# Sohojoe/ppo-dash

Measured on AMD Instinct MI355X. Metric: env-steps/sec (rollout+GAE+PPO update) at 4096 envs×128 steps, 1/2/4/8 MI355X, higher is better.
Workload: dtype f32

## Files before the change

### ppo-dash_amd/csrc/gemm.hip

```cpp
#include "igemm.h"
#include "igemm_x9.h"
#include "small.h"

namespace {
constexpr int IMG = 84, IMG2 = 84 * 84;
constexpr int C1S = 7104;
static_assert(C1S >= IMG2 && (C1S / 2) % 64 == 32, "conv1 stage channel stride");

template <typename InT, class C_>
struct Conv1Fwd : C_ {
  using BCtx = typename C_::BCtx;
  const InT* obs; const int64_t* idx; long long row0; int C, M;
  const float* w; const float* bias; float* out;
  struct ACtx { const InT* base; bool ok; };
  __device__ ACtx a_ctx(int m, int) const {
    if (m >= M) return {obs, false};
    const int b = m / 400, pp = m - b * 400, oy = pp / 20, ox = pp - oy * 20;
    return {obs + obs_row(idx, row0, b) * (long long)(C * IMG2) + (oy * 4) * IMG + ox * 4, true};
  }
  using Raw = std::conditional_t<sizeof(InT) == 1, uint32_t, f32x4>;
  __device__ Raw a_load(const ACtx& c, int k) const {
    if (!c.ok) return Raw{};
    const int ch = k >> 6, ky = (k >> 3) & 7, kx = k & 7;
    return *reinterpret_cast<const Raw*>(c.base + ch * IMG2 + ky * IMG + kx);
// ... 401 lines not shown
__device__ __forceinline__ void conv2_fwd_x9c_body(const float* __restrict__ a1, int B,
                                                   const uint16_t* __restrict__ wpl, const float* __restrict__ bias,
                                                   float* __restrict__ out, uint16_t* __restrict__ mbits,
                                                   uint8_t* __restrict__ lds) {
  constexpr int U = 400, PLN = 4 * U, STG = 3 * PLN, KS = 8, WN = 64 * 512;
  static_assert(MT == 5 || MT == 6, "row tiles: 6, or 5 with the lone pixel elsewhere");
  constexpr int UNITS = 4 * U, UPER = (UNITS + 511) / 512;
  static_assert(STG == C2F_STG, "stage size");
  bf16x8* const S = reinterpret_cast<bf16x8*>(lds);
  int (*const vtab)[16] = reinterpret_cast<int (*)[16]>(lds + 2 * STG * 16);
  int (*const otab)[16] = reinterpret_cast<int (*)[16]>(lds + 2 * STG * 16 + MT * 16 * 4);
  const int tid = threadIdx.x, lane = tid & 63, wave = tid >> 6, i16 = lane & 15, g = lane >> 4;
  const int nt = wave & 3, kh = wave >> 2, co = 16 * nt + i16;
  if (tid < 16) {
    int t = 0;
    for (int v = tid; v <= 88; v += 16)
      if (v % 10 != 9 && t < MT) {
        vtab[t][tid] = v;
        otab[t][tid] = 9 * (v / 10) + v % 10;
        ++t;
      }
    if (MT == 5 && t == 4) {
      const int v = 82 + (tid - 9);
      vtab[4][tid] = v;
      otab[4][tid] = 9 * (v / 10) + v % 10;
      t = 5;
    }
    for (; t < MT; ++t) {
      vtab[t][tid] = tid;
      otab[t][tid] = -1;
    }
  }
  bf16x8 bw[KS][3];
#pragma unroll
  for (int s = 0; s < KS; ++s)
#pragma unroll
    for (int p = 0; p < 3; ++p)
      bw[s][p] = *reinterpret_cast<const bf16x8*>(wpl + (size_t)p * WN + co * 512 + (8 * kh + s) * 32 + 8 * g);
  const f32x4 bv4 = *reinterpret_cast<const f32x4*>(bias + 16 * nt + 4 * g);
  wait_vm0();
  int usrc[UPER], udst[UPER];
#pragma unroll
  for (int j = 0; j < UPER; ++j) {
    const int u = min(tid + 512 * j, UNITS - 1), rho = 8 * (u >> 5) + (u & 7), c = (u >> 3) & 3;
    const int par = rho / 100, rem = rho - 100 * par, yh = rem / 10, xh = rem - 10 * yh;
    const int y = 2 * yh + (par >> 1), x = 2 * xh + (par & 1);
    usrc[j] = (y * 20 + x) * 8 + 2 * c;
    udst[j] = c * U + rho;
  }
  const bool has_last = tid + 512 * (UPER - 1) < UNITS;
  f32x4 stg[UPER][2];
  bf16x8 lo[UPER];
  auto fetch_unit = [&](int b, int j) {
    if constexpr ((DBG & 4) != 0) {
      asm volatile("" : "+v"(stg[j][0]), "+v"(stg[j][1]));
      return;
    }
    const f32x4* src = reinterpret_cast<const f32x4*>(a1 + (size_t)b * 12800);
    stg[j][0] = src[usrc[j]];
    stg[j][1] = src[usrc[j] + 1];
  };
  auto fetch = [&](int b) {
#pragma unroll
    for (int j = 0; j < UPER; ++j) fetch_unit(b, j);
  };
  auto put_hm = [&](int j, int st) {
    if constexpr ((DBG & 2) != 0) {
      asm volatile("" ::"v"(stg[j][0]), "v"(stg[j][1]));
      return;
    }
    Frag3 f;
    split8(stg[j][0], stg[j][1], f, NP == 1);
    lo[j] = f.l;
    if (j < UPER - 1 || has_last) {
      bf16x8* d = S + st * STG + udst[j];
      d[0] = f.h;
      if constexpr (NP > 1) d[PLN] = f.m;
    }
  };
  auto put_l = [&](int j, int st) {
    if constexpr ((DBG & 2) != 0) return;
    if constexpr (NP > 1)
      if (j < UPER - 1 || has_last) S[st * STG + 2 * PLN + udst[j]] = lo[j];
  };
  auto lds_barrier = []() { asm volatile("s_waitcnt lgkmcnt(0)\n\ts_barrier" ::: "memory"); };
  __syncthreads();
  int vrow[MT];
#pragma unroll
  for (int t = 0; t < MT; ++t) vrow[t] = vtab[t][i16] + g * U;
  const int G = gridDim.x;
  int b = blockIdx.x, cur = 0;
  if (b < B) {
    fetch(b);
#pragma unroll
    for (int j = 0; j < UPER; ++j) {
      put_hm(j, 0);
      put_l(j, 0);
    }
    fetch(b + G < B ? b + G : b);
  }
  __syncthreads();
  for (; b < B; b += G) {
    const int bnn = b + 2 * G < B ? b + 2 * G : b;
    const bf16x8* Sc = S + cur * STG;
    f32x4 acc[MT];
#pragma unroll
    for (int t = 0; t < MT; ++t) acc[t] = zero4();
#pragma unroll
    for (int s = 0; s < KS; ++s) {
      const int tap = 8 * kh + s, ky = tap >> 2, kx = tap & 3;
      const int toff = 100 * (2 * (ky & 1) + (kx & 1)) + 10 * (ky >> 1) + (kx >> 1);
      const Frag3 w = {bw[s][0], bw[s][1], bw[s][2]};
#pragma unroll
      for (int t0 = 0; t0 < MT; t0 += 3) {
        Frag3 a[3];
#pragma unroll
        for (int u = 0; u < 3; ++u) {
          if (t0 + u >= MT) continue;
          const bf16x8* q = Sc + vrow[t0 + u] + toff;
          a[u].h = q[0];
          if constexpr (NP > 1) {
            a[u].m = q[PLN];
            a[u].l = q[2 * PLN];
          }
        }
#define PPO_PART(X, Y) \
  _Pragma("unroll") for (int u = 0; u < 3; ++u) if (t0 + u < MT) acc[t0 + u] = mma(w.Y, a[u].X, acc[t0 + u]);
        if constexpr ((DBG & 1) == 0) {
          PPO_PRODUCTS(NP, PPO_PART)
        } else {
#pragma unroll
          for (int u = 0; u < 3; ++u)
            if (t0 + u < MT) asm volatile("" ::"v"(a[u].h), "v"(a[u].m), "v"(a[u].l));
        }
#undef PPO_PART
      }
      if (s < UPER) put_hm(s, cur ^ 1);
      if (s >= 1 && s <= UPER) fetch_unit(bnn, s - 1);
      if (s == 5) lds_barrier();
      if (s >= 6) {
#pragma unroll
        for (int j = 0; j < UPER; ++j)
          if ((j & 1) == s - 6) put_l(j, cur ^ 1);
      }
    }
    lds_barrier();
    f32x4* R = reinterpret_cast<f32x4*>(S + cur * STG + 2 * PLN);
    if (kh == 1) {
#pragma unroll
      for (int t = 0; t < MT; ++t) R[(nt * MT + t) * 64 + lane] = acc[t];
    }
    lds_barrier();
    if (kh == 0) {
      const auto rs = make_rsrc(out + (size_t)b * (81 * 64), 81 * 64 * 4);
#pragma unroll
      for (int t = 0; t < MT; ++t) {
        const f32x4 v = acc[t] + R[(nt * MT + t) * 64 + lane];
        const int m = otab[t][i16];
        f32x4 y;
#pragma unroll
        for (int r = 0; r < 4; ++r) y[r] = fmaxf(v[r] + bv4[r], 0.f);
        if constexpr ((DBG & 8) == 0) bstore_f32x4(y, rs, m >= 0 ? 4 * (m * 64 + 16 * nt + 4 * g) : -1);
        if constexpr (MASK && (DBG & 8) == 0) {
          int nib = 0;
#pragma unroll
          for (int r = 0; r < 4; ++r) nib |= (y[r] > 0.f ? 1 : 0) << r;
          const int w16 = nib | (__shfl_down(nib, 16, 64) << 4) | (__shfl_down(nib, 32, 64) << 8) |
                          (__shfl_down(nib, 48, 64) << 12);
          if (g == 0 && m >= 0) mbits[((size_t)b * 81 + m) * 4 + nt] = (uint16_t)w16;
        }
      }
    }
    cur ^= 1;
  }
  if constexpr (MT == 5 && LONE) {
    __syncthreads();
    const int blk = blockIdx.x;
    const int nimg = blk < B ? (B - 1 - blk) / G + 1 : 0;
    conv2_lone_tiles<NP, MASK>(a1, bw, bias, out, mbits, lds, blk, G, nimg, 0, 1);
  }
}

#ifndef C2F_LONE
#define C2F_LONE 1
#endif
template <int NP, bool MASK = false, int DBG = 0>
__global__ __launch_bounds__(512) void conv2_fwd_x9c_kernel(const float* __restrict__ a1, int B,
                                                           const uint16_t* __restrict__ wpl,
                                                           const float* __restrict__ bias,
                                                           float* __restrict__ out,
                                                           uint16_t* __restrict__ mbits) {
  __shared__ __attribute__((aligned(16))) uint8_t lds[C2F_LDS];
  conv2_fwd_x9c_body<NP, MASK, DBG, C2F_LONE ? 5 : 6, C2F_LONE == 2>(a1, B, wpl, bias, out, mbits, lds);
}

constexpr int C2L_IR = 65;
constexpr int C2L_PL = 16 * C2L_IR;
constexpr int C2L_LDS = 2 * 3 * C2L_PL * 16 + 4 * 64 * 16;
static_assert(C2L_LDS <= C2F_LDS, "the lone tiles reuse the image loop's LDS");
template <int NP, bool MASK>
__device__ __forceinline__ void conv2_lone_tiles(const float* __restrict__ a1, const bf16x8 (&bw)[8][3],
                                                 const float* __restrict__ bias, float* __restrict__ out,
                                                 uint16_t* __restrict__ mbits, uint8_t* __restrict__ lds,
                                                 long long base, long long stride, int nimg, int t0, int tstep) {
  constexpr int KS = 8, M = 72, IR = C2L_IR, PL = C2L_PL;
  uint4 (*const P)[3 * PL] = reinterpret_cast<uint4 (*)[3 * PL]>(lds);
  f32x4* const R = reinterpret_cast<f32x4*>(lds + 2 * 3 * PL * 16);
  const int tid = threadIdx.x, lane = tid & 63, i16 = lane & 15, g = lane >> 4;
  const int wave = __builtin_amdgcn_readfirstlane(tid >> 6);
  const int nt = wave & 3, kh = wave >> 2;
  const int ntile = (nimg + 15) / 16;
  f32x4 pc[2][2];
  auto fetch = [&](int T) {
#pragma unroll
    for (int j = 0; j < 2; ++j) {
      const int c = tid + 512 * j, im = c >> 6, u = c & 63, i = 16 * T + im;
      const bool live = T < ntile && i < nimg;
      const float* src = a1 + (size_t)(base + stride * (live ? i : 0)) * 12800 + (16 + (u >> 4)) * 640 + (u & 15) * 8;
      pc[j][0] = live ? *reinterpret_cast<const f32x4*>(src) : zero4();
      pc[j][1] = live ? *reinterpret_cast<const f32x4*>(src + 4) : zero4();
    }
  };
  auto put = [&](int st) {
#pragma unroll
    for (int j = 0; j < 2; ++j) {
      const int c = tid + 512 * j, o = (c >> 6) * IR + (c & 63);
      Frag3 f;
      split8(pc[j][0], pc[j][1], f, NP == 1);
      P[st][o] = __builtin_bit_cast(uint4, f.h);
      if constexpr (NP != 1) {
        P[st][PL + o] = __builtin_bit_cast(uint4, f.m);
        P[st][2 * PL + o] = __builtin_bit_cast(uint4, f.l);
      }
    }
  };
  fetch(t0);
  put(0);
  __syncthreads();
  int cur = 0;
  for (int T = t0; T < ntile; T += tstep) {
    fetch(T + tstep);
    const int i = 16 * T + i16;
    const bool live = i < nimg;
    const long long b = base + stride * (long long)i;
    f32x4 acc = zero4();
#pragma unroll
    for (int s = 0; s < KS; ++s) {
      const int o = i16 * IR + (8 * kh + s) * 4 + g;
      Frag3 a;
      a.h = __builtin_bit_cast(bf16x8, P[cur][o]);
      if constexpr (NP != 1) {
        a.m = __builtin_bit_cast(bf16x8, P[cur][PL + o]);
        a.l = __builtin_bit_cast(bf16x8, P[cur][2 * PL + o]);
      }
      const Frag3 w = {bw[s][0], bw[s][1], bw[s][2]};
#define PPO_PART(X, Y) acc = mma(w.Y, a.X, acc);
      PPO_PRODUCTS(NP, PPO_PART)
#undef PPO_PART
    }
    if (kh == 1) R[nt * 64 + lane] = acc;
    put(cur ^ 1);
    __syncthreads();
    if (kh == 0) {
      const f32x4 bv4 = *reinterpret_cast<const f32x4*>(bias + 16 * nt + 4 * g);
      const f32x4 v = acc + R[nt * 64 + lane];
      f32x4 y;
#pragma unroll
      for (int r = 0; r < 4; ++r) y[r] = fmaxf(v[r] + bv4[r], 0.f);
      if (live) *reinterpret_cast<f32x4*>(out + (size_t)b * (81 * 64) + M * 64 + 16 * nt + 4 * g) = y;
      if constexpr (MASK) {
        int nib = 0;
#pragma unroll
        for (int r = 0; r < 4; ++r) nib |= (y[r] > 0.f ? 1 : 0) << r;
        const int w16 = nib | (__shfl_down(nib, 16, 64) << 4) | (__shfl_down(nib, 32, 64) << 8) |
                        (__shfl_down(nib, 48, 64) << 12);
        if (g == 0 && live) mbits[((size_t)b * 81 + M) * 4 + nt] = (uint16_t)w16;
      }
    }
    __syncthreads();
    cur ^= 1;
  }
}

template <int NP, bool MASK>
__global__ __launch_bounds__(512) void conv2_fwd_lone_kernel(const float* __restrict__ a1, int B,
                                                             const uint16_t* __restrict__ wpl,
                                                             const float* __restrict__ bias,
                                                             float* __restrict__ out,
                                                             uint16_t* __restrict__ mbits) {
  constexpr int KS = 8, WN = 64 * 512;
  __shared__ __attribute__((aligned(16))) uint8_t lds[C2L_LDS];
  const int tid = threadIdx.x, i16 = tid & 15, g = (tid & 63) >> 4, wave = tid >> 6;
  const int co = 16 * (wave & 3) + i16, kh = wave >> 2;
  bf16x8 bw[KS][3];
#pragma unroll
  for (int s = 0; s < KS; ++s)
#pragma unroll
    for (int p = 0; p < 3; ++p)
      bw[s][p] = *reinterpret_cast<const bf16x8*>(wpl + (size_t)p * WN + co * 512 + (8 * kh + s) * 32 + 8 * g);
  conv2_lone_tiles<NP, MASK>(a1, bw, bias, out, mbits, lds, 0, 1, B, blockIdx.x, gridDim.x);
}

__device__ __forceinline__ int c2w_pix(int r) {
  r = r < 80 ? r : 80;
  return r < 72 ? (r >> 3) * 9 + (r & 7) : (r - 72) * 9 + 8;
}

template <int NP, int DBG = 0>
__global__ __launch_bounds__(512) void conv2_wgrad_x9_kernel(const float* __restrict__ dz2,
                                                            const float* __restrict__ a1, int B,
                                                            float* __restrict__ slab,
                                                            float* __restrict__ slab_bias) {
  constexpr int XPL = 400 * 32, DR = 112, DPL = 64 * DR;
  constexpr int XU = 1600, XPER = (XU + 511) / 512, DU = 64 * 12, DPER = (DU + 511) / 512;
  __shared__ __attribute__((aligned(16))) uint16_t X[3 * XPL];
  __shared__ __attribute__((aligned(16))) uint16_t D[3 * DPL];
  __shared__ float bred[512];
  const int tid = threadIdx.x, lane = tid & 63, wave = tid >> 6, i16 = lane & 15, g = lane >> 4;
  const int q = i16 >> 2, p = i16 & 3;
  int Qb[3][2];
#pragma unroll
  for (int s = 0; s < 3; ++s)
#pragma unroll
    for (int h = 0; h < 2; ++h) {
      const int m = c2w_pix(32 * s + 8 * g + 4 * h + q), oy = m / 9;
      Qb[s][h] = 40 * oy + (m - 9 * oy);
    }
  int xsrc[XPER], xdst[XPER];
#pragma unroll
  for (int j = 0; j < XPER; ++j) {
    const int u = tid + 512 * j, Q = u >> 2, c = u & 3, y = Q / 20, rem = Q - 20 * y;
    const int x = rem < 10 ? 2 * rem : 2 * (rem - 10) + 1;
    xsrc[j] = (y * 20 + x) * 32 + 8 * c;
    xdst[j] = Q * 32 + 8 * (c ^ (((Q >> 3) & 1) * 2));
  }
  f32x4 xs[XPER][2];
  float ds[DPER][8];
  float bsum = 0.f;
  auto fetch_part = [&](int b, int k) {
    if constexpr ((DBG & 4) != 0) return;
    if (k < 4) {
      const auto ra = make_rsrc(a1 + (size_t)b * 12800, 12800 * 4);
      const int off = tid + 512 * k < XU ? xsrc[k] * 4 : 0x7ffffff0;
      xs[k][0] = __builtin_bit_cast(f32x4, __builtin_amdgcn_raw_buffer_load_b128(ra, off, 0, 0));
      xs[k][1] = __builtin_bit_cast(f32x4, __builtin_amdgcn_raw_buffer_load_b128(ra, off + 16, 0, 0));
    } else {
      const auto rd = make_rsrc(dz2 + (size_t)b * (81 * 64), 81 * 64 * 4);
      const int j = (k - 4) >> 1, e0 = 4 * ((k - 4) & 1), v = tid + 512 * j;
#pragma unroll
      for (int e = e0; e < e0 + 4; ++e) {
        const int r = 8 * (v >> 6) + e;
        const int off = v < DU && r < 81 ? (c2w_pix(r) * 64 + (v & 63)) * 4 : 0x7ffffff0;
        ds[j][e] = __builtin_bit_cast(float, __builtin_amdgcn_raw_buffer_load_b32(rd, off, 0, 0));
      }
    }
  };
  auto fetch = [&](int b) {
#pragma unroll
    for (int k = 0; k < 8; ++k) fetch_part(b, k);
  };
  auto put = [&](bool count) {
    if constexpr ((DBG & 2) != 0) return;
#pragma unroll
    for (int j = 0; j < XPER; ++j)
      if (tid + 512 * j < XU) {
        Frag3 f;
        split8(xs[j][0], xs[j][1], f, false);
        *reinterpret_cast<bf16x8*>(&X[xdst[j]]) = f.h;
        *reinterpret_cast<bf16x8*>(&X[XPL + xdst[j]]) = f.m;
        *reinterpret_cast<bf16x8*>(&X[2 * XPL + xdst[j]]) = f.l;
      }
#pragma unroll
    for (int j = 0; j < DPER; ++j) {
      const int v = tid + 512 * j;
      if (v < DU) {
        Frag3 f;
        split8(f32x4{ds[j][0], ds[j][1], ds[j][2], ds[j][3]}, f32x4{ds[j][4], ds[j][5], ds[j][6], ds[j][7]}, f,
               false);
#pragma unroll
        for (int e = 0; e < 8; ++e) bsum += count ? ds[j][e] : 0.f;
        const int off = (v & 63) * DR + 8 * (v >> 6);
        *reinterpret_cast<bf16x8*>(&D[off]) = f.h;
        *reinterpret_cast<bf16x8*>(&D[DPL + off]) = f.m;
        *reinterpret_cast<bf16x8*>(&D[2 * DPL + off]) = f.l;
      }
    }
  };
  f32x4 acc[4][4];
#pragma unroll
  for (int j = 0; j < 4; ++j)
#pragma unroll
    for (int mt = 0; mt < 4; ++mt) acc[j][mt] = zero4();
  const int Z = gridDim.x;
  int b = blockIdx.x;
  if ((DBG & 16) == 0 && (blockIdx.x & 1)) __builtin_amdgcn_s_sleep(100);
  if (b < B) {
    fetch(b);
    put(true);
  }
  __syncthreads();
  typedef short s16x4 __attribute__((ext_vector_type(4)));
  for (; b < B; b += Z) {
    const bool pf = b + Z < B;
    const int bn = pf ? b + Z : b;
#pragma unroll
    for (int s = 0; s < 3; ++s) {
      Frag3 a[4];
#pragma unroll
      for (int mt = 0; mt < 4; ++mt) {
        const int off = (16 * mt + i16) * DR + 32 * s + 8 * g;
        a[mt].h = *reinterpret_cast<const bf16x8*>(&D[off]);
        a[mt].m = *reinterpret_cast<const bf16x8*>(&D[DPL + off]);
        a[mt].l = *reinterpret_cast<const bf16x8*>(&D[2 * DPL + off]);
      }
#pragma unroll
      for (int j = 0; j < 4; ++j) {
        if constexpr ((DBG & 8) != 0) {
#pragma unroll
          for (int k = 0; k < 8; ++k)
            if ((3 * k) >> 1 == 4 * s + j) {
              fetch_part(bn, k);
              __builtin_amdgcn_sched_barrier(0);
            }
        } else if (4 * s + j < 8) {
          fetch_part(bn, 4 * s + j);
          __builtin_amdgcn_sched_barrier(0);
        }
        const int tap = 2 * wave + (j >> 1), ky = tap >> 2, kx = tap & 3, cb = j & 1;
        const int toff = 20 * ky + 10 * (kx & 1) + (kx >> 1);
        s16x4 t[3][2];
#pragma unroll
        for (int h = 0; h < 2; ++h) {
          const int Q = Qb[s][h] + toff, unit = (4 * cb + p) ^ (((Q >> 3) & 1) * 4);
          const uint16_t* rp = &X[Q * 32 + 4 * unit];
#pragma unroll
          for (int pl = 0; pl < 3; ++pl)
            t[pl][h] = __builtin_amdgcn_ds_read_tr16_b64_v4i16(
                (__attribute__((address_space(3))) s16x4*)(rp + pl * XPL));
        }
        Frag3 bf;
        bf.h = __builtin_bit_cast(bf16x8, __builtin_shufflevector(t[0][0], t[0][1], 0, 1, 2, 3, 4, 5, 6, 7));
        bf.m = __builtin_bit_cast(bf16x8, __builtin_shufflevector(t[1][0], t[1][1], 0, 1, 2, 3, 4, 5, 6, 7));
        bf.l = __builtin_bit_cast(bf16x8, __builtin_shufflevector(t[2][0], t[2][1], 0, 1, 2, 3, 4, 5, 6, 7));
#define PPO_PART(XX, YY) \
  _Pragma("unroll") for (int mt = 0; mt < 4; ++mt) acc[j][mt] = mma(a[mt].XX, bf.YY, acc[j][mt]);
        if constexpr ((DBG & 1) == 0) {
          PPO_PRODUCTS(NP, PPO_PART)
        } else {
#pragma unroll
          for (int mt = 0; mt < 4; ++mt) acc[j][mt][0] += (float)a[mt].h[0] + (float)bf.h[0] + (float)bf.l[1];
        }
#undef PPO_PART
      }
    }
    __syncthreads();
    put(pf);
    __syncthreads();
  }
  float* o = slab + (size_t)blockIdx.x * (64 * 512) + 64 * wave + i16;
#pragma unroll
  for (int j = 0; j < 4; ++j)
#pragma unroll
    for (int mt = 0; mt < 4; ++mt)
#pragma unroll
      for (int r = 0; r < 4; ++r) o[(16 * mt + 4 * g + r) * 512 + 16 * j] = acc[j][mt][r];
  bred[tid] = bsum;
  __syncthreads();
  if (tid < 64) {
    float t = 0.f;
#pragma unroll
    for (int w = 0; w < 8; ++w) t += bred[tid + 64 * w];
    slab_bias[(size_t)blockIdx.x * 64 + tid] = t;
  }
}

template <int NP, bool BITS = false>
__global__ __launch_bounds__(512) void conv3_dgrad_x9_kernel(const float* __restrict__ dz3, int B,
                                                            const uint16_t* __restrict__ wpl,
                                                            const float* __restrict__ a2,
                                                            float* __restrict__ dz2, int stagger) {
  constexpr int GW = 25, CS = 288, PLU = 4 * CS, KS = 9, WN = 64 * 288;
  constexpr int DU = 49 * 4, MC = 81 * 64 / 4, MPER = (MC + 511) / 512;
  __shared__ __attribute__((aligned(16))) uint16_t S[2][3 * PLU * 8];
  __shared__ __attribute__((aligned(16))) uint32_t Mk[2][MC];
  const int tid = threadIdx.x, lane = tid & 63, wave = tid >> 6, i16 = lane & 15, g = lane >> 4;
  const int nt = wave & 3, mh = wave >> 2, ci = 16 * nt + i16;
  bf16x8 bw[KS][3];
#pragma unroll
  for (int s = 0; s < KS; ++s)
#pragma unroll
    for (int p = 0; p < 3; ++p)
      bw[s][p] = *reinterpret_cast<const bf16x8*>(wpl + (size_t)p * WN + ci * 288 + 32 * s + 8 * g);
  wait_vm0();
  for (int i = tid; i < 2 * 3 * PLU; i += 512) reinterpret_cast<uint4*>(&S[0][0])[i] = uint4{0, 0, 0, 0};
  constexpr unsigned TILES = 0x430521u;
  int qrow[3], tl[3];
#pragma unroll
  for (int t = 0; t < 3; ++t) {
    tl[t] = (TILES >> (4 * (3 * mh + t))) & 15;
    const int m = min(16 * tl[t] + i16, 80), y = m / 9, x = m - 9 * y;
    qrow[t] = g * CS + (y + 2) * GW + x + 2;
  }
  f32x4 stg[2];
  f32x4 mst[BITS ? 1 : MPER];
  uint2 mbv;
  auto fetch = [&](int b) {
    if (tid < DU) {
      const f32x4* src = reinterpret_cast<const f32x4*>(dz3 + (size_t)b * 1568);
      stg[0] = src[2 * tid];
      stg[1] = src[2 * tid + 1];
    }
    if constexpr (BITS) {
      if (tid < 81) mbv = reinterpret_cast<const uint2*>(a2)[(size_t)b * 81 + tid];
    } else {
      const f32x4* ms = reinterpret_cast<const f32x4*>(a2 + (size_t)b * 5184);
#pragma unroll
      for (int j = 0; j < MPER; ++j)
        if (tid + 512 * j < MC) mst[j] = ms[tid + 512 * j];
    }
  };
  auto put = [&](int buf) {
    if (tid < DU) {
      const int px = tid >> 2, oy = px / 7, ox = px - 7 * oy;
      const int q = (tid & 3) * CS + (oy + 2) * GW + ox + 2;
      Frag3 f;
      split8(stg[0], stg[1], f, false);
      *reinterpret_cast<bf16x8*>(&S[buf][8 * q]) = f.h;
      *reinterpret_cast<bf16x8*>(&S[buf][8 * (PLU + q)]) = f.m;
      *reinterpret_cast<bf16x8*>(&S[buf][8 * (2 * PLU + q)]) = f.l;
    }
    if constexpr (BITS) {
      if (tid < 81) reinterpret_cast<uint2*>(Mk[buf])[tid] = mbv;
    } else {
#pragma unroll
      for (int j = 0; j < MPER; ++j) {
        const int c = tid + 512 * j;
        if (c < MC)
          Mk[buf][c] = (mst[j][0] > 0.f ? 1u : 0u) | (mst[j][1] > 0.f ? 0x100u : 0u) |
                       (mst[j][2] > 0.f ? 0x10000u : 0u) | (mst[j][3] > 0.f ? 0x1000000u : 0u);
      }
    }
  };
  __syncthreads();
  const int G = gridDim.x;
  int b = blockIdx.x, cur = 0;
  if (b < B) {
    fetch(b);
    put(0);
    if (b + G < B) fetch(b + G);
  }
  __syncthreads();
  const bool late = stagger && wave >= 4;
  for (; b < B; b += G) {
    if (!late) {
      if (b + G < B) put(cur ^ 1);
      if (b + 2 * G < B) fetch(b + 2 * G);
    }
    const uint16_t* Sc = S[cur];
    f32x4 acc[3];
#pragma unroll
    for (int t = 0; t < 3; ++t) acc[t] = zero4();
    auto compute = [&](auto M0, auto M1, auto M2) {
      constexpr unsigned msk[3] = {decltype(M0)::value, decltype(M1)::value, decltype(M2)::value};
#pragma unroll
      for (int s = 0; s < KS; ++s) {
        const int toff = -(GW * (s / 3) + s % 3);
        const Frag3 w = {bw[s][0], bw[s][1], bw[s][2]};
        Frag3 a[3];
#pragma unroll
        for (int u = 0; u < 3; ++u) {
          if (!((msk[u] >> s) & 1u)) continue;
          const uint16_t* q = Sc + 8 * (qrow[u] + toff);
          a[u].h = *reinterpret_cast<const bf16x8*>(q);
          a[u].m = *reinterpret_cast<const bf16x8*>(q + 8 * PLU);
          a[u].l = *reinterpret_cast<const bf16x8*>(q + 16 * PLU);
        }
#define PPO_PART(X, Y) \
  _Pragma("unroll") for (int u = 0; u < 3; ++u) if ((msk[u] >> s) & 1u) acc[u] = mma(w.Y, a[u].X, acc[u]);
        PPO_PRODUCTS(NP, PPO_PART)
#undef PPO_PART
      }
    };
    using std::integral_constant;
    if (mh == 0)
      compute(integral_constant<unsigned, 0x1FF>{}, integral_constant<unsigned, 0x1FF>{},
              integral_constant<unsigned, 0x100>{});
    else
      compute(integral_constant<unsigned, 0x03F>{}, integral_constant<unsigned, 0x1FF>{},
              integral_constant<unsigned, 0x1F8>{});
    const uint8_t* mk = reinterpret_cast<const uint8_t*>(Mk[cur]);
    const auto rs = make_rsrc(dz2 + (size_t)b * 5184, 5184 * 4);
    const int c0 = 16 * nt + 4 * g;
#pragma unroll
    for (int t = 0; t < 3; ++t) {
      const int m = 16 * tl[t] + i16, mm = min(m, 80);
      const uint32_t mw = Mk[cur][2 * mm + (c0 >> 5)] >> (c0 & 31);
      f32x4 y;
#pragma unroll
      for (int r = 0; r < 4; ++r) {
        const bool keep = BITS ? ((mw >> r) & 1u) != 0 : mk[mm * 64 + c0 + r] != 0;
        y[r] = keep ? acc[t][r] : 0.f;
      }
      bstore_f32x4(y, rs, m < 81 ? 4 * (m * 64 + c0) : -1);
    }
    if (late) {
      if (b + G < B) put(cur ^ 1);
      if (b + 2 * G < B) fetch(b + 2 * G);
    }
    __syncthreads();
    cur ^= 1;
  }
}

constexpr int C3F_PL = 84 * 64;
constexpr int C3F_LDS = 2 * 3 * C3F_PL * 2 + 2 * 2 * 2 * 2 * 64 * 16;
template <int NP>
__device__ __forceinline__ void conv3_fwd_x9_body(const float* __restrict__ a2, int B,
                                                  const uint16_t* __restrict__ wpl, const float* __restrict__ bias,
                                                  float* __restrict__ out, uint8_t* __restrict__ lds) {
  constexpr int NPX = 84, PL = NPX * 64, KS = 9, WN = 32 * 576, UNITS = 81 * 8, UPER = (UNITS + 511) / 512;
  static_assert(PL == C3F_PL, "plane size");
  uint16_t (*const S)[3 * PL] = reinterpret_cast<uint16_t (*)[3 * PL]>(lds);
  f32x4 (*const R)[2][2][2][64] = reinterpret_cast<f32x4 (*)[2][2][2][64]>(lds + 2 * 3 * PL * 2);
  const int tid = threadIdx.x, lane = tid & 63, wave = tid >> 6, i16 = lane & 15, g = lane >> 4;
  const int nt = wave & 1, kh = (wave >> 1) & 1, mh = wave >> 2, co = 16 * nt + i16;
  bf16x8 bw[KS][3];
#pragma unroll
  for (int s = 0; s < KS; ++s)
#pragma unroll
    for (int p = 0; p < 3; ++p)
      bw[s][p] = *reinterpret_cast<const bf16x8*>(wpl + (size_t)p * WN + co * 576 + (9 * kh + s) * 32 + 8 * g);
  const f32x4 bv4 = *reinterpret_cast<const f32x4*>(bias + 16 * nt + 4 * g);
  wait_vm0();
  for (int i = tid; i < 2 * 3 * PL / 8; i += 512) reinterpret_cast<uint4*>(&S[0][0])[i] = uint4{0, 0, 0, 0};
  f32x4 stg[UPER][2];
  auto fetch_unit = [&](int b, int j) {
    const auto ra = make_rsrc(a2 + (size_t)b * 5184, 5184 * 4);
    const int u = tid + 512 * j, off = u < UNITS ? 32 * u : 0x7fffffe0;
    stg[j][0] = __builtin_bit_cast(f32x4, __builtin_amdgcn_raw_buffer_load_b128(ra, off, 0, 0));
    stg[j][1] = __builtin_bit_cast(f32x4, __builtin_amdgcn_raw_buffer_load_b128(ra, off + 16, 0, 0));
  };
  auto fetch = [&](int b) {
#pragma unroll
    for (int j = 0; j < UPER; ++j) fetch_unit(b, j);
  };
  auto put = [&](int buf) {
#pragma unroll
    for (int j = 0; j < UPER; ++j) {
      const int u = tid + 512 * j;
      if (u < UNITS) {
        const int p = u >> 3, off = p * 64 + 8 * ((u & 7) ^ ((p >> 1) & 7));
        Frag3 f;
        split8(stg[j][0], stg[j][1], f, false);
        *reinterpret_cast<bf16x8*>(&S[buf][off]) = f.h;
        *reinterpret_cast<bf16x8*>(&S[buf][PL + off]) = f.m;
        *reinterpret_cast<bf16x8*>(&S[buf][2 * PL + off]) = f.l;
      }
    }
  };
  __syncthreads();
  const int G = gridDim.x;
  int b = blockIdx.x, cur = 0;
  if (b < B) {
    fetch(b);
    put(0);
    fetch(b + G < B ? b + G : b);
  }
  __syncthreads();
  for (; b < B; b += G) {
    put(cur ^ 1);
    const int bnn = b + 2 * G < B ? b + 2 * G : b;
    const uint16_t* Sc = S[cur];
    f32x4 acc[2] = {zero4(), zero4()};
#pragma unroll
    for (int s = 0; s < KS; ++s) {
      const int ks = 9 * kh + s, tap = ks >> 1, ky = tap / 3, kx = tap - 3 * ky, c = 4 * (ks & 1) + g;
      const Frag3 w = {bw[s][0], bw[s][1], bw[s][2]};
      Frag3 a[2];
#pragma unroll
      for (int u = 0; u < 2; ++u) {
        const int p = 16 * (2 * mh + u) + i16 + 9 * ky + kx;
        const uint16_t* q = Sc + p * 64 + 8 * (c ^ ((p >> 1) & 7));
        a[u].h = *reinterpret_cast<const bf16x8*>(q);
        a[u].m = *reinterpret_cast<const bf16x8*>(q + PL);
        a[u].l = *reinterpret_cast<const bf16x8*>(q + 2 * PL);
      }
#define PPO_PART(X, Y) \
  _Pragma("unroll") for (int u = 0; u < 2; ++u) acc[u] = mma(w.Y, a[u].X, acc[u]);
      PPO_PRODUCTS(NP, PPO_PART)
#undef PPO_PART
      if (s == 1 || s == 3) {
        fetch_unit(bnn, s >> 1);
        __builtin_amdgcn_sched_barrier(0);
      }
    }
    if (kh == 1) {
      R[cur][nt][mh][0][lane] = acc[0];
      R[cur][nt][mh][1][lane] = acc[1];
    }
    __syncthreads();
    if (kh == 0) {
      const auto rs = make_rsrc(out + (size_t)b * (49 * 32), 49 * 32 * 4);
#pragma unroll
      for (int u = 0; u < 2; ++u) {
        const f32x4 v = acc[u] + R[cur][nt][mh][u][lane];
        const int m = 16 * (2 * mh + u) + i16, oy = m / 9, ox = m - 9 * oy;
        f32x4 y;
#pragma unroll
        for (int r = 0; r < 4; ++r) y[r] = fmaxf(v[r] + bv4[r], 0.f);
        bstore_f32x4(y, rs, (ox < 7 && oy < 7) ? 4 * ((7 * oy + ox) * 32 + 16 * nt + 4 * g) : -1);
      }
    }
    cur ^= 1;
  }
}

template <int NP>
__global__ __launch_bounds__(512) void conv3_fwd_x9_kernel(const float* __restrict__ a2, int B,
                                                          const uint16_t* __restrict__ wpl,
                                                          const float* __restrict__ bias,
                                                          float* __restrict__ out, int stagger) {
  __shared__ __attribute__((aligned(16))) uint8_t lds[C3F_LDS];
  (void)stagger;
  conv3_fwd_x9_body<NP>(a2, B, wpl, bias, out, lds);
}

constexpr int C3L_IR = 73;
constexpr int C3L_PL = 16 * C3L_IR;
constexpr int C3L_LDS = 2 * 3 * C3L_PL * 16 + 2 * 64 * 16;
constexpr int C3C_LDS0 = 2 * 3 * 84 * 80 * 2 + 2 * 2 * 3 * 64 * 16;
constexpr int C3C_LDS = C3C_LDS0 > C3L_LDS ? C3C_LDS0 : C3L_LDS;

constexpr int C3_LONE_Y = 6, C3_LONE_X = 0, C3_LONE_Q = 7 * C3_LONE_Y + C3_LONE_X;
__constant__ uint8_t c3_row_q[48] = {0,  1,  2,  3,  20, 7,  8,  9,  10, 11, 12, 19, 4,  5,  6,  13,
                                     26, 27, 14, 15, 32, 33, 34, 21, 22, 23, 24, 31, 16, 17, 18, 25,
                                     38, 39, 40, 41, 44, 45, 46, 47, 48, 35, 36, 43, 28, 29, 30, 37};

__device__ __forceinline__ void conv3_mask_store(const f32x4& y, int g, uint16_t* dst) {
  uint32_t w = ((y[0] > 0.f ? 1u : 0u) | (y[1] > 0.f ? 2u : 0u) | (y[2] > 0.f ? 4u : 0u) | (y[3] > 0.f ? 8u : 0u))
               << (4 * g);
  w |= (uint32_t)__shfl_xor((int)w, 16, 64);
  w |= (uint32_t)__shfl_xor((int)w, 32, 64);
  if (g == 0) *dst = (uint16_t)w;
}

template <int NP, int NT>
__device__ __forceinline__ void conv3_lone_tiles(const float* __restrict__ a2, const bf16x8 (&bw)[9][3],
                                                 const float* __restrict__ bias, float* __restrict__ out,
                                                 uint8_t* __restrict__ lds, long long base, long long stride,
                                                 int nimg, int t0, int tstep, uint16_t* __restrict__ m3 = nullptr) {
  constexpr int KS = 9, M = C3_LONE_Q, IR = C3L_IR, PL = C3L_PL, NCH = 16 * 72, NPC = (NCH + NT - 1) / NT;
  uint4 (*const P)[3 * PL] = reinterpret_cast<uint4 (*)[3 * PL]>(lds);
  f32x4* const R = reinterpret_cast<f32x4*>(lds + 2 * 3 * PL * 16);
  const int tid = threadIdx.x, lane = tid & 63, i16 = lane & 15, g = lane >> 4;
  const int wave = __builtin_amdgcn_readfirstlane(tid >> 6);
  const int nt = wave & 1, kh = (wave >> 1) & 1;
  const int ntile = (nimg + 15) / 16;
  f32x4 pc[NPC][2];
  auto fetch = [&](int T) {
// ... 1400 lines not shown
```

Baseline: 1.568 million.

## Pair conv2 wgrad tail pixels across image pairs and batch the lone pixel

The conv2 weight-gradient kernel used to run a third K-step of 32 pixels per image, only 17 of which were valid (81 = 64+17). The rewrite packs the 16-pixel tails of two consecutive images into one K-step by alternating a position slot, so the third step runs every other image. The lone 81st pixel is handled in a separate phase that batches 32 images per MMA. This cuts wasted MFMA work on padding, but adds LDS space, extra duplicated stores, zero-initialisation and a second fetch loop with more indexing complexity.

```diff
diff --git a/ppo-dash_amd/csrc/gemm.hip b/ppo-dash_amd/csrc/gemm.hip
--- a/ppo-dash_amd/csrc/gemm.hip
+++ b/ppo-dash_amd/csrc/gemm.hip
@@ -727,17 +727,17 @@
 }
 
 __device__ __forceinline__ int c2w_pix(int r) {
-  r = r < 80 ? r : 80;
-  return r < 72 ? (r >> 3) * 9 + (r & 7) : (r - 72) * 9 + 8;
-}
-
-template <int NP, int DBG = 0>
+  return r < 56 ? (r >> 3) * 9 + (r & 7) : r < 64 ? (r - 56) * 9 + 8 : 63 + (r - 64) + ((r - 64) >> 3);
+}
+
+template <int NP>
 __global__ __launch_bounds__(512) void conv2_wgrad_x9_kernel(const float* __restrict__ dz2,
                                                             const float* __restrict__ a1, int B,
                                                             float* __restrict__ slab,
                                                             float* __restrict__ slab_bias) {
-  constexpr int XPL = 400 * 32, DR = 112, DPL = 64 * DR;
-  constexpr int XU = 1600, XPER = (XU + 511) / 512, DU = 64 * 12, DPER = (DU + 511) / 512;
+  constexpr int XPL = 520 * 32, TQ0 = 280, TQD = 120, DR = 112, DPL = 64 * DR;
+  constexpr int XU = 1600, XPER = (XU + 511) / 512, DU = 64 * 10, DPER = (DU + 511) / 512;
+  static_assert(XPL >= 32 * 512, "the lone phase's [32 images][512] plane fits an X plane");
   __shared__ __attribute__((aligned(16))) uint16_t X[3 * XPL];
   __shared__ __attribute__((aligned(16))) uint16_t D[3 * DPL];
   __shared__ float bred[512];
@@ -748,22 +748,22 @@
   for (int s = 0; s < 3; ++s)
 #pragma unroll
     for (int h = 0; h < 2; ++h) {
-      const int m = c2w_pix(32 * s + 8 * g + 4 * h + q), oy = m / 9;
-      Qb[s][h] = 40 * oy + (m - 9 * oy);
-    }
-  int xsrc[XPER], xdst[XPER];
+      const int m = c2w_pix(s < 2 ? 32 * s + 8 * g + 4 * h + q : 64 + 8 * (g & 1) + 4 * h + q), oy = m / 9;
+      Qb[s][h] = 40 * oy + (m - 9 * oy) + (s == 2 && g < 2 ? TQD : 0);
+    }
+  int xsrc[XPER], xdst[XPER], xdt[XPER];
 #pragma unroll
   for (int j = 0; j < XPER; ++j) {
     const int u = tid + 512 * j, Q = u >> 2, c = u & 3, y = Q / 20, rem = Q - 20 * y;
     const int x = rem < 10 ? 2 * rem : 2 * (rem - 10) + 1;
     xsrc[j] = (y * 20 + x) * 32 + 8 * c;
     xdst[j] = Q * 32 + 8 * (c ^ (((Q >> 3) & 1) * 2));
+    xdt[j] = Q >= TQ0 && Q < 400 ? (Q + TQD) * 32 + 8 * (c ^ ((((Q + TQD) >> 3) & 1) * 2)) : -1;
   }
   f32x4 xs[XPER][2];
   float ds[DPER][8];
   float bsum = 0.f;
   auto fetch_part = [&](int b, int k) {
-    if constexpr ((DBG & 4) != 0) return;
     if (k < 4) {
       const auto ra = make_rsrc(a1 + (size_t)b * 12800, 12800 * 4);
       const int off = tid + 512 * k < XU ? xsrc[k] * 4 : 0x7ffffff0;
@@ -775,7 +775,7 @@
 #pragma unroll
       for (int e = e0; e < e0 + 4; ++e) {
         const int r = 8 * (v >> 6) + e;
-        const int off = v < DU && r < 81 ? (c2w_pix(r) * 64 + (v & 63)) * 4 : 0x7ffffff0;
+        const int off = v < DU ? (c2w_pix(r) * 64 + (v & 63)) * 4 : 0x7ffffff0;
         ds[j][e] = __builtin_bit_cast(float, __builtin_amdgcn_raw_buffer_load_b32(rd, off, 0, 0));
       }
     }
@@ -784,8 +784,7 @@
 #pragma unroll
     for (int k = 0; k < 8; ++k) fetch_part(b, k);
   };
-  auto put = [&](bool count) {
-    if constexpr ((DBG & 2) != 0) return;
+  auto put = [&](bool count, int pos) {
 #pragma unroll
     for (int j = 0; j < XPER; ++j)
       if (tid + 512 * j < XU) {
@@ -794,6 +793,11 @@
         *reinterpret_cast<bf16x8*>(&X[xdst[j]]) = f.h;
         *reinterpret_cast<bf16x8*>(&X[XPL + xdst[j]]) = f.m;
         *reinterpret_cast<bf16x8*>(&X[2 * XPL + xdst[j]]) = f.l;
+        if (512 * j + 511 >= 4 * TQ0 && pos == 0 && xdt[j] >= 0) {
+          *reinterpret_cast<bf16x8*>(&X[xdt[j]]) = f.h;
+          *reinterpret_cast<bf16x8*>(&X[XPL + xdt[j]]) = f.m;
+          *reinterpret_cast<bf16x8*>(&X[2 * XPL + xdt[j]]) = f.l;
+        }
       }
 #pragma unroll
     for (int j = 0; j < DPER; ++j) {
@@ -804,7 +808,7 @@
                false);
 #pragma unroll
         for (int e = 0; e < 8; ++e) bsum += count ? ds[j][e] : 0.f;
-        const int off = (v & 63) * DR + 8 * (v >> 6);
+        const int sg = v >> 6, off = (v & 63) * DR + 8 * sg + (sg >= 8 ? 16 * pos : 0);
         *reinterpret_cast<bf16x8*>(&D[off]) = f.h;
         *reinterpret_cast<bf16x8*>(&D[DPL + off]) = f.m;
         *reinterpret_cast<bf16x8*>(&D[2 * DPL + off]) = f.l;
@@ -818,68 +822,130 @@
     for (int mt = 0; mt < 4; ++mt) acc[j][mt] = zero4();
   const int Z = gridDim.x;
   int b = blockIdx.x;
-  if ((DBG & 16) == 0 && (blockIdx.x & 1)) __builtin_amdgcn_s_sleep(100);
+  if (blockIdx.x & 1) __builtin_amdgcn_s_sleep(100);
+  for (int i = tid; i < 3 * 64 * 2; i += 512)
+    *reinterpret_cast<uint4*>(&D[(i >> 1) * DR + 64 + 8 * (i & 1)]) = uint4{0, 0, 0, 0};
+  for (int i = tid; i < 3 * TQD * 4; i += 512) {
+    const int pl = i / (TQD * 4);
+    *reinterpret_cast<uint4*>(&X[pl * XPL + 400 * 32 + 8 * (i - pl * TQD * 4)]) = uint4{0, 0, 0, 0};
+  }
+  __syncthreads();
+  const int nimg = b < B ? (B - 1 - b) / Z + 1 : 0;
+  int pos = nimg & 1;
   if (b < B) {
     fetch(b);
-    put(true);
+    put(true, pos);
   }
   __syncthreads();
   typedef short s16x4 __attribute__((ext_vector_type(4)));
+  Frag3 a[4];
+  auto load_a = [&](int d0) {
+#pragma unroll
+    for (int mt = 0; mt < 4; ++mt) {
+      const int off = (16 * mt + i16) * DR + d0 + 8 * g;
+      a[mt].h = *reinterpret_cast<const bf16x8*>(&D[off]);
+      a[mt].m = *reinterpret_cast<const bf16x8*>(&D[DPL + off]);
+      a[mt].l = *reinterpret_cast<const bf16x8*>(&D[2 * DPL + off]);
+    }
+  };
+  auto mma_tile = [&](int j, const uint16_t* rp0, const uint16_t* rp1) {
+    s16x4 t[3][2];
+#pragma unroll
+    for (int pl = 0; pl < 3; ++pl) {
+      t[pl][0] = __builtin_amdgcn_ds_read_tr16_b64_v4i16((__attribute__((address_space(3))) s16x4*)(rp0 + pl * XPL));
+      t[pl][1] = __builtin_amdgcn_ds_read_tr16_b64_v4i16((__attribute__((address_space(3))) s16x4*)(rp1 + pl * XPL));
+    }
+    Frag3 bf;
+    bf.h = __builtin_bit_cast(bf16x8, __builtin_shufflevector(t[0][0], t[0][1], 0, 1, 2, 3, 4, 5, 6, 7));
+    bf.m = __builtin_bit_cast(bf16x8, __builtin_shufflevector(t[1][0], t[1][1], 0, 1, 2, 3, 4, 5, 6, 7));
+    bf.l = __builtin_bit_cast(bf16x8, __builtin_shufflevector(t[2][0], t[2][1], 0, 1, 2, 3, 4, 5, 6, 7));
+#define PPO_PART(XX, YY) \
+  _Pragma("unroll") for (int mt = 0; mt < 4; ++mt) acc[j][mt] = mma(a[mt].XX, bf.YY, acc[j][mt]);
+    PPO_PRODUCTS(NP, PPO_PART)
+#undef PPO_PART
+  };
   for (; b < B; b += Z) {
     const bool pf = b + Z < B;
     const int bn = pf ? b + Z : b;
 #pragma unroll
-    for (int s = 0; s < 3; ++s) {
-      Frag3 a[4];
-#pragma unroll
-      for (int mt = 0; mt < 4; ++mt) {
-        const int off = (16 * mt + i16) * DR + 32 * s + 8 * g;
-        a[mt].h = *reinterpret_cast<const bf16x8*>(&D[off]);
-        a[mt].m = *reinterpret_cast<const bf16x8*>(&D[DPL + off]);
-        a[mt].l = *reinterpret_cast<const bf16x8*>(&D[2 * DPL + off]);
-      }
-#pragma unroll
-      for (int j = 0; j < 4; ++j) {
-        if constexpr ((DBG & 8) != 0) {
-#pragma unroll
-          for (int k = 0; k < 8; ++k)
-            if ((3 * k) >> 1 == 4 * s + j) {
-              fetch_part(bn, k);
-              __builtin_amdgcn_sched_barrier(0);
-            }
-        } else if (4 * s + j < 8) {
-          fetch_part(bn, 4 * s + j);
-          __builtin_amdgcn_sched_barrier(0);
+    for (int s = 0; s < 3; ++s)
+      if (s < 2 || pos) {
+        load_a(32 * s);
+#pragma unroll
+        for (int j = 0; j < 4; ++j) {
+          if (s < 2) {
+            fetch_part(bn, 4 * s + j);
+            __builtin_amdgcn_sched_barrier(0);
+          }
+          const int tap = 2 * wave + (j >> 1), ky = tap >> 2, kx = tap & 3, cb = j & 1;
+          const int toff = 20 * ky + 10 * (kx & 1) + (kx >> 1);
+          const uint16_t* rp[2];
+#pragma unroll
+          for (int h = 0; h < 2; ++h) {
+            const int Q = Qb[s][h] + toff, unit = (4 * cb + p) ^ (((Q >> 3) & 1) * 4);
+            rp[h] = &X[Q * 32 + 4 * unit];
+          }
+          mma_tile(j, rp[0], rp[1]);
         }
-        const int tap = 2 * wave + (j >> 1), ky = tap >> 2, kx = tap & 3, cb = j & 1;
-        const int toff = 20 * ky + 10 * (kx & 1) + (kx >> 1);
-        s16x4 t[3][2];
-#pragma unroll
-        for (int h = 0; h < 2; ++h) {
-          const int Q = Qb[s][h] + toff, unit = (4 * cb + p) ^ (((Q >> 3) & 1) * 4);
-          const uint16_t* rp = &X[Q * 32 + 4 * unit];
-#pragma unroll
-          for (int pl = 0; pl < 3; ++pl)
-            t[pl][h] = __builtin_amdgcn_ds_read_tr16_b64_v4i16(
-                (__attribute__((address_space(3))) s16x4*)(rp + pl * XPL));
-        }
-        Frag3 bf;
-        bf.h = __builtin_bit_cast(bf16x8, __builtin_shufflevector(t[0][0], t[0][1], 0, 1, 2, 3, 4, 5, 6, 7));
-        bf.m = __builtin_bit_cast(bf16x8, __builtin_shufflevector(t[1][0], t[1][1], 0, 1, 2, 3, 4, 5, 6, 7));
-        bf.l = __builtin_bit_cast(bf16x8, __builtin_shufflevector(t[2][0], t[2][1], 0, 1, 2, 3, 4, 5, 6, 7));
-#define PPO_PART(XX, YY) \
-  _Pragma("unroll") for (int mt = 0; mt < 4; ++mt) acc[j][mt] = mma(a[mt].XX, bf.YY, acc[j][mt]);
-        if constexpr ((DBG & 1) == 0) {
-          PPO_PRODUCTS(NP, PPO_PART)
-        } else {
-#pragma unroll
-          for (int mt = 0; mt < 4; ++mt) acc[j][mt][0] += (float)a[mt].h[0] + (float)bf.h[0] + (float)bf.l[1];
-        }
-#undef PPO_PART
-      }
-    }
+      }
     __syncthreads();
-    put(pf);
+    pos ^= 1;
+    put(pf, pos);
+    __syncthreads();
+  }
+  auto lone_fetch = [&](int n0) {
+#pragma unroll
+    for (int j = 0; j < 4; ++j) {
+      const int n = n0 + __builtin_amdgcn_readfirstlane(wave) + 8 * j;
+      const auto ra = make_rsrc(a1 + (size_t)(blockIdx.x + (n < nimg ? n : 0) * (long long)Z) * 12800, 12800 * 4);
+      const int px = lane >> 2, off = n < nimg ? (((16 + (px >> 2)) * 20 + 16 + (px & 3)) * 32 + 8 * (lane & 3)) * 4
+                                               : 0x7ffffff0;
+      xs[j][0] = __builtin_bit_cast(f32x4, __builtin_amdgcn_raw_buffer_load_b128(ra, off, 0, 0));
+      xs[j][1] = __builtin_bit_cast(f32x4, __builtin_amdgcn_raw_buffer_load_b128(ra, off + 16, 0, 0));
+    }
+#pragma unroll
+    for (int e = 0; e < 8; ++e) {
+      const int n = n0 + 8 * __builtin_amdgcn_readfirstlane(wave) + e;
+      const auto rd = make_rsrc(dz2 + (size_t)(blockIdx.x + (n < nimg ? n : 0) * (long long)Z) * (81 * 64), 81 * 64 * 4);
+      const int off = wave < 4 && n < nimg ? (80 * 64 + lane) * 4 : 0x7ffffff0;
+      ds[0][e] = __builtin_bit_cast(float, __builtin_amdgcn_raw_buffer_load_b32(rd, off, 0, 0));
+    }
+  };
+  auto lone_put = [&]() {
+#pragma unroll
+    for (int j = 0; j < 4; ++j) {
+      Frag3 f;
+      split8(xs[j][0], xs[j][1], f, false);
+      const int i = wave + 8 * j, off = i * 512 + 4 * ((8 * (lane >> 2) + 2 * (lane & 3)) ^ (4 * (i & 3)));
+      *reinterpret_cast<bf16x8*>(&X[off]) = f.h;
+      *reinterpret_cast<bf16x8*>(&X[XPL + off]) = f.m;
+      *reinterpret_cast<bf16x8*>(&X[2 * XPL + off]) = f.l;
+    }
+    if (wave < 4) {
+      Frag3 f;
+      split8(f32x4{ds[0][0], ds[0][1], ds[0][2], ds[0][3]}, f32x4{ds[0][4], ds[0][5], ds[0][6], ds[0][7]}, f, false);
+#pragma unroll
+      for (int e = 0; e < 8; ++e) bsum += ds[0][e];
+      const int off = lane * DR + 8 * wave;
+      *reinterpret_cast<bf16x8*>(&D[off]) = f.h;
+      *reinterpret_cast<bf16x8*>(&D[DPL + off]) = f.m;
+      *reinterpret_cast<bf16x8*>(&D[2 * DPL + off]) = f.l;
+    }
+  };
+  if (nimg > 0) lone_fetch(0);
+  for (int n0 = 0; n0 < nimg; n0 += 32) {
+    lone_put();
+    __syncthreads();
+    if (n0 + 32 < nimg) lone_fetch(n0 + 32);
+    load_a(0);
+#pragma unroll
+    for (int j = 0; j < 4; ++j) {
+      const int tap = 2 * wave + (j >> 1), cb = j & 1;
+      const uint16_t* rp[2];
+#pragma unroll
+      for (int h = 0; h < 2; ++h) rp[h] = &X[(8 * g + 4 * h + q) * 512 + 4 * ((8 * tap + 4 * cb + p) ^ (4 * q))];
+      mma_tile(j, rp[0], rp[1]);
+    }
     __syncthreads();
   }
   float* o = slab + (size_t)blockIdx.x * (64 * 512) + 64 * wave + i16;
```

Result: no change. 1.579 million, median of 6 (+0.7%).
